# vlc-robot/robot-3dlotus

Hardware: AMD Instinct MI355X
Metric: keystep-samples/sec (train fwd+bwd) 3D-LOTUS GemBench (higher is better)
Workload: dtype f32; 1 GPU; 3D-LOTUS v1 (68.18M params), 16 key-step clouds x 4096 pts per GPU, fwd+loss+bwd, train mode (dropout on), fp32 exact (MFMA f32); global_batch=16, parallelism=dp1, rccl_ranks=0

## Files before the change

### robot-3dlotus_amd/csrc/conv.hip

```cpp
#include "mma.h"

namespace LOTUS_NS {

int lotus_reduce_parts(const float* part, float* out, long n, long stride, int nz, int accumulate, hipStream_t st);
int lotus_conv_pairs_try(int mode, const act_t* x, const float* w, const float* w_t, const float* bias, const act_t* add,
                         act_t* y, const int* nbr, const int* rowidx, int n, int T, int cin, int cout, void* workspace,
                         size_t workspace_bytes, int prec, hipStream_t st, int* rc);
size_t lotus_conv_pairs_workspace(int n, int ND);
int lotus_conv_weight_transpose_impl(const float* w, float* wt, int cout, int T, int cin, int prec, hipStream_t st);
int lotus_conv_tap_gemm(int mode, const act_t* x, const float* w, float* part, const int* tg_in, const int* tg_cnt, int n64,
                        int src_rows, int cin, int cout, hipStream_t st);

static int tap_min_width() {
  static int v = -1;
  if (v < 0) { const char* e = getenv("LOTUS_CONV_TAP_MINC"); v = e ? atoi(e) : 64; }
  return v;
}
static size_t tap_slab_max() {
  static long v = -1;
  if (v < 0) { const char* e = getenv("LOTUS_CONV_TAP_SLAB_MB"); v = e ? atol(e) : 2047; }
  return (size_t)v << 20;
}
static size_t tap_part_bytes(int n, int ND);
static bool tap_shape_ok(int n, int cin, int cout) {
// ... 386 lines not shown
      if (b_fast) rrb[e] = ldraw(p.x + (long)max(qq, 0) * p.cin + ci0 + iq * 4);
      else rrb[e] = toraw(load4_guard(p.x, p.cin, max(qq, 0), ci0 + iq * 4, p.n, p.cin, b_vec), p.x);
    }
  };
  auto stage = [&](unsigned* W, int plane, const float4& v0, const float4& v1, bool sum) __attribute__((always_inline)) {
    const float va[4] = {v0.x, v0.y, v0.z, v0.w}, vb[4] = {v1.x, v1.y, v1.z, v1.w};
    unsigned hw[4], lw[4];
#pragma unroll
    for (int e = 0; e < 4; ++e) split_bf16(va[e], vb[e], hw[e], lw[e]);
    if (sum) {
#pragma unroll
      for (int e = 0; e < 4; ++e) bsum[e] += va[e] + vb[e];
    }
    const int rot = (iq >> 2) & 3;
    rot4(hw, rot);
    if (PREC == 3) rot4(lw, rot);
#pragma unroll
    for (int e = 0; e < 4; ++e) {
      const int row = iq * 4 + ((e + rot) & 3);
      W[row * TA::kLdW + kr2] = hw[e];
      if (PREC == 3) W[plane + row * TA::kLdW + kr2] = lw[e];
    }
  };
  auto lstore = [&]() __attribute__((always_inline)) {
    stage(Aw, TA::kPlaneW, zsel4(oka[0], unraw(rra[0])), zsel4(oka[1], unraw(rra[1])), want_bias);
    stage(Bw, TB::kPlaneW, zsel4(okb[0], unraw(rrb[0])), zsel4(okb[1], unraw(rrb[1])), false);
  };
  if (total > 0) {
    gload(0);
    lstore();
    __syncthreads();
    for (int k0 = 0; k0 < total; k0 += BK) {
      const bool more = k0 + BK < total;
      if (more) gload(k0 + BK);
      gemm_slab_bf16<BM, BN, BK, PREC>(Aw, Bw, wr0, wc0, acc);
      __syncthreads();
      if (more) {
        lstore();
        __syncthreads();
      }
    }
  }
  float* part = p.part + (long)blockIdx.z * p.part_stride;
  const int col = ci0 + acc_col(wc0, 0);
  if (col < p.cin) {
#pragma unroll
    for (int r = 0; r < 16; ++r) {
      const int row = co0 + acc_row(wr0, 0, r);
      if (row < p.cout) part[((long)row * p.T + t) * p.cin + col] = acc[0][0][r];
    }
  }
  if (want_bias) {
    float4* red = reinterpret_cast<float4*>(Aw);
    red[tid] = make_float4(bsum[0], bsum[1], bsum[2], bsum[3]);
    __syncthreads();
    if (tid < BM) {
      float s = 0.f;
#pragma unroll
      for (int g = 0; g < 16; ++g) {
        const float4 v = red[g * 16 + (tid >> 2)];
        s += (tid & 3) == 0 ? v.x : (tid & 3) == 1 ? v.y : (tid & 3) == 2 ? v.z : v.w;
      }
      if (co0 + tid < p.cout) p.bias_part[(long)blockIdx.z * p.part_stride + co0 + tid] = s;
    }
  }
}

static size_t conv_dyn_lds(int T, int BM) { return (size_t)(T * BM + 2 * T) * sizeof(int); }

extern "C" {

size_t lotus_subm_conv_workspace(int n, int cin, int cout) {
  const size_t a = lotus_conv_pairs_workspace(n, cout), b = lotus_conv_pairs_workspace(n, cin);
  const size_t c = tap_shape_ok(n, cin, cout) ? tap_part_bytes(n, cin > cout ? cin : cout) : 0;
  const size_t ab = a > b ? a : b;
  return ab > c ? ab : c;
}
int lotus_conv_tap_eligible(int n, int cin, int cout) {
  static int on = -1;
  if (on < 0) { const char* e = getenv("LOTUS_CONV_TAP"); on = (e && e[0] == '0') ? 0 : 1; }
  return on && tap_shape_ok(n, cin, cout) ? 1 : 0;
}

#define STEM_ROWS 32
#define STEM_TP 128

}

__global__ void conv_stem_wt_kernel(const float* __restrict__ w, float* __restrict__ wt, int cout, int T, int cin) {
  const int i = blockIdx.x * blockDim.x + threadIdx.x;
  if (i >= cout * T * cin) return;
  const int c = i % cout, rem = i / cout;
  wt[i] = w[(long)c * T * cin + rem];
}

template <int CIN>
__global__ __launch_bounds__(256) void conv_smallcin_kernel(ConvP p) {
  __shared__ int list_nb[STEM_ROWS * STEM_TP];
  __shared__ unsigned char list_t[STEM_ROWS * STEM_TP];
  __shared__ int cnt_s[STEM_ROWS];
  const int tid = threadIdx.x, r = tid >> 3, j = tid & 7;
  const int m = blockIdx.y * STEM_ROWS + r, cb = blockIdx.x;
  const bool valid = m < p.n;
  {
    int nbv[16];
    unsigned flags = 0;
#pragma unroll
    for (int k = 0; k < 16; ++k) {
      const int t = 16 * j + k;
      nbv[k] = (valid && t < p.T) ? p.nbr[(long)t * p.n + m] : -1;
      flags |= (nbv[k] >= 0 ? 1u : 0u) << k;
    }
    const int mine = __popc(flags);
    int incl = mine;
#pragma unroll
    for (int o = 1; o < 8; o <<= 1) {
      const int v = __shfl_up(incl, o, 8);
      if (j >= o) incl += v;
    }
    int pos = incl - mine;
    if (j == 7) cnt_s[r] = incl;
#pragma unroll
    for (int k = 0; k < 16; ++k)
      if (flags & (1u << k)) {
        list_t[r * STEM_TP + pos] = (unsigned char)(16 * j + k);
        list_nb[r * STEM_TP + pos] = nbv[k];
        ++pos;
      }
  }
  float acc[8];
#pragma unroll
  for (int k = 0; k < 8; ++k) acc[k] = p.bias ? p.bias[cb * 64 + j * 8 + k] : 0.f;
  __syncthreads();
  const int len = cnt_s[r];
  const float* wbase = p.w + cb * 64 + j * 8;
  const int cin = CIN ? CIN : p.cin;
  int t = 0;
  float xl = 0.f;
  if (len > 0) {
    t = list_t[r * STEM_TP];
    xl = j < cin ? p.x[(long)list_nb[r * STEM_TP] * cin + j] : 0.f;
  }
  for (int cur = 0; cur < len; ++cur) {
    const float* wr = wbase + (long)t * cin * p.cout;
    const float xc = xl;
    if (cur + 1 < len) {
      t = list_t[r * STEM_TP + cur + 1];
      xl = j < cin ? p.x[(long)list_nb[r * STEM_TP + cur + 1] * cin + j] : 0.f;
    }
    if (CIN) {
      float4 w0[CIN ? CIN : 1], w1[CIN ? CIN : 1];
#pragma unroll
      for (int ci = 0; ci < CIN; ++ci) {
        w0[ci] = ld4(wr + ci * p.cout);
        w1[ci] = ld4(wr + ci * p.cout + 4);
      }
#pragma unroll
      for (int ci = 0; ci < CIN; ++ci) {
        const float xv = __shfl(xc, ci, 8);
        acc[0] = fmaf(xv, w0[ci].x, acc[0]); acc[1] = fmaf(xv, w0[ci].y, acc[1]); acc[2] = fmaf(xv, w0[ci].z, acc[2]); acc[3] = fmaf(xv, w0[ci].w, acc[3]);
        acc[4] = fmaf(xv, w1[ci].x, acc[4]); acc[5] = fmaf(xv, w1[ci].y, acc[5]); acc[6] = fmaf(xv, w1[ci].z, acc[6]); acc[7] = fmaf(xv, w1[ci].w, acc[7]);
      }
    } else {
      for (int ci = 0; ci < cin; ++ci) {
        const float4 w0 = ld4(wr + ci * p.cout);
        const float4 w1 = ld4(wr + ci * p.cout + 4);
        const float xv = __shfl(xc, ci, 8);
        acc[0] = fmaf(xv, w0.x, acc[0]); acc[1] = fmaf(xv, w0.y, acc[1]); acc[2] = fmaf(xv, w0.z, acc[2]); acc[3] = fmaf(xv, w0.w, acc[3]);
        acc[4] = fmaf(xv, w1.x, acc[4]); acc[5] = fmaf(xv, w1.y, acc[5]); acc[6] = fmaf(xv, w1.z, acc[6]); acc[7] = fmaf(xv, w1.w, acc[7]);
      }
    }
  }
  if (valid) {
    act_t* yo = p.y + (long)m * p.ND + cb * 64 + j * 8;
    if (p.add) {
      const act_t* ao = p.add + (long)m * p.ND + cb * 64 + j * 8;
#pragma unroll
      for (int k = 0; k < 8; ++k) acc[k] += ao[k];
    }
    st4(yo, make_float4(acc[0], acc[1], acc[2], acc[3]));
    st4(yo + 4, make_float4(acc[4], acc[5], acc[6], acc[7]));
  }
}

extern "C" {

int lotus_conv_weight_transpose(const float* w, float* w_t, int cout, int T, int cin, int precision, void* stream) {
  LOTUS_CHECK_ARG(w && w_t && cout > 0 && T > 0 && cin > 0, "lotus_conv_weight_transpose: bad arguments");
  LOTUS_CHECK_ARG(precision == 0 || precision == 1 || precision == 3, "lotus_conv_weight_transpose: precision must be 0, 1 or 3");
  return lotus_conv_weight_transpose_impl(w, w_t, cout, T, cin, precision, (hipStream_t)stream);
}

int lotus_subm_conv(int mode, const act_t* x, const float* w, const float* w_t, const float* bias, const act_t* add,
                    act_t* y, const int* nbr, const int* rowidx, int n, int T, int cin, int cout, int precision,
                    const int* tap_plan, void* workspace, size_t workspace_bytes, void* stream) {
  LOTUS_CHECK_ARG(x && w && y && nbr && n >= 0 && T > 0 && cin > 0 && cout > 0, "lotus_subm_conv: bad arguments");
  LOTUS_CHECK_ARG(precision == 0 || precision == 1 || precision == 3, "lotus_subm_conv: precision must be 0, 1 or 3");
  if (n == 0) return LOTUS_OK;
  if (tap_plan && T == 27 && precision == 0 && lotus_conv_tap_eligible(n, cin, cout)) {
    LOTUS_CHECK_ARG(workspace && ((uintptr_t)workspace) % 16 == 0 && workspace_bytes >= tap_part_bytes(n, mode == 0 ? cout : cin),
                    "lotus_subm_conv: the tap-grouped path needs a 16-byte aligned workspace of lotus_subm_conv_workspace(n, cin, cout) bytes");
    LOTUS_CHECK_ARG((((uintptr_t)x) | ((uintptr_t)w) | ((uintptr_t)y) | ((uintptr_t)bias) | ((uintptr_t)add)) % 16 == 0,
                    "lotus_subm_conv: the tap-grouped path needs 16-byte aligned operands");
    const int n64 = (n + 63) / 64 * 64, ND = mode == 0 ? cout : cin;
    const int rc = lotus_conv_tap_gemm(mode, x, w, (float*)workspace, tap_plan + 32, tap_plan, n64, n, cin, cout, (hipStream_t)stream);
    if (rc != LOTUS_OK) return rc;
    const long total4 = (long)n * ND / 4;
    const int g = (int)cdiv(total4, 256);
    LOTUS_LAUNCH(conv_tap_reduce_kernel, dim3(g > 4096 ? 4096 : g), dim3(256), 0, (hipStream_t)stream, (const float*)workspace,
                 tap_plan + 32 + 27L * n64, n, ND, bias, add, y);
    LOTUS_LAUNCH_CHECK("lotus_subm_conv(tap-grouped)");
    return LOTUS_OK;
  }
  {
    int rc = 0;
    if (lotus_conv_pairs_try(mode, x, w, w_t, bias, add, y, nbr, rowidx, n, T, cin, cout, workspace, workspace_bytes,
                             precision, (hipStream_t)stream, &rc))
      return rc;
  }
  ConvP p;
  memset(&p, 0, sizeof(p));
  p.x = x; p.w = w; p.y = y; p.bias = bias; p.add = add; p.nbr = nbr; p.rowidx = rowidx;
  p.n = n; p.T = T; p.cin = cin; p.cout = cout;
  p.KD = mode == 0 ? cin : cout;
  p.ND = mode == 0 ? cout : cin;
  p.mirror = mode == 1;
  hipStream_t st = (hipStream_t)stream;
  if (mode == 0 && cin <= 8 && cout % 64 == 0 && T <= STEM_TP && ((uintptr_t)y) % 16 == 0 && workspace &&
      ((uintptr_t)workspace) % 16 == 0 && workspace_bytes >= (size_t)T * cin * cout * sizeof(float)) {
    LOTUS_LAUNCH(conv_stem_wt_kernel, dim3(cdiv((long)cout * T * cin, 256)), dim3(256), 0, st, w, (float*)workspace, cout, T,
                       cin);
    p.w = (const float*)workspace;
    const dim3 sg(cout / 64, cdiv(n, STEM_ROWS));
    if (cin == 7) LOTUS_LAUNCH((conv_smallcin_kernel<7>), sg, dim3(256), 0, st, p);
    else if (cin == 8) LOTUS_LAUNCH((conv_smallcin_kernel<8>), sg, dim3(256), 0, st, p);
    else if (cin == 6) LOTUS_LAUNCH((conv_smallcin_kernel<6>), sg, dim3(256), 0, st, p);
    else if (cin == 4) LOTUS_LAUNCH((conv_smallcin_kernel<4>), sg, dim3(256), 0, st, p);
    else LOTUS_LAUNCH((conv_smallcin_kernel<0>), sg, dim3(256), 0, st, p);
    LOTUS_LAUNCH_CHECK("lotus_subm_conv(stem)");
    return LOTUS_OK;
  }
  dim3 block(256);
  const size_t dyn = conv_dyn_lds(T, 128);
  LOTUS_CHECK_ARG(dyn + 20000 <= 160 * 1024, "lotus_subm_conv: %d taps do not fit LDS", T);
  if (p.ND <= 64) {
    dim3 grid(cdiv(p.ND, 64), cdiv(n, 128));
    if (mode == 0) {
      { static bool a1 = false; if (!a1) { (void)hipFuncSetAttribute((const void*)conv_kernel<128, 64, true>, hipFuncAttributeMaxDynamicSharedMemorySize, (int)dyn); a1 = true; } }
      LOTUS_LAUNCH((conv_kernel<128, 64, true>), grid, block, dyn, st, p);
    } else {
      { static bool a2 = false; if (!a2) { (void)hipFuncSetAttribute((const void*)conv_kernel<128, 64, false>, hipFuncAttributeMaxDynamicSharedMemorySize, (int)dyn); a2 = true; } }
      LOTUS_LAUNCH((conv_kernel<128, 64, false>), grid, block, dyn, st, p);
    }
  } else {
    dim3 grid(cdiv(p.ND, 128), cdiv(n, 128));
    if (mode == 0) {
      { static bool a3 = false; if (!a3) { (void)hipFuncSetAttribute((const void*)conv_kernel<128, 128, true>, hipFuncAttributeMaxDynamicSharedMemorySize, (int)dyn); a3 = true; } }
      LOTUS_LAUNCH((conv_kernel<128, 128, true>), grid, block, dyn, st, p);
    } else {
      { static bool a4 = false; if (!a4) { (void)hipFuncSetAttribute((const void*)conv_kernel<128, 128, false>, hipFuncAttributeMaxDynamicSharedMemorySize, (int)dyn); a4 = true; } }
      LOTUS_LAUNCH((conv_kernel<128, 128, false>), grid, block, dyn, st, p);
    }
  }
  LOTUS_LAUNCH_CHECK("lotus_subm_conv");
  return LOTUS_OK;
}

static __global__ __launch_bounds__(256) void conv_smallcin_wgrad_kernel(ConvWgP p) {
  constexpr int NW = WG_MAX_PAIRS / 256, SB = 512;
  __shared__ int prow_s[WG_MAX_PAIRS];
  __shared__ int pnb_s[WG_MAX_PAIRS];
  __shared__ __attribute__((aligned(16))) float xs[SB][8];
  __shared__ float red[4][64][8];
  __shared__ int wcnt[NW][4];
  const int tid = threadIdx.x, c = tid & 63, g = tid >> 6, lane = tid & 63;
  const int cb = blockIdx.x, t = blockIdx.y, z = blockIdx.z;
  const int rbeg = z * p.chunk, rend = min(p.n, rbeg + p.chunk);
  int total = 0;
  {
    int nbv[NW];
    unsigned long long mv[NW];
#pragma unroll
    for (int w = 0; w < NW; ++w) {
      const int row = rbeg + w * 256 + tid;
      nbv[w] = row < rend ? p.nbr[(long)t * p.n + row] : -1;
    }
#pragma unroll
    for (int w = 0; w < NW; ++w) {
      mv[w] = __ballot(nbv[w] >= 0);
      if (lane == 0) wcnt[w][g] = __popcll(mv[w]);
    }
    __syncthreads();
#pragma unroll
    for (int w = 0; w < NW; ++w) {
      int base = total;
#pragma unroll
      for (int q = 0; q < 4; ++q) {
        if (q < g) base += wcnt[w][q];
        total += wcnt[w][q];
      }
      if (nbv[w] >= 0) {
        const int pos = base + __popcll(mv[w] & ((1ull << lane) - 1ull));
        prow_s[pos] = rbeg + w * 256 + tid;
        pnb_s[pos] = nbv[w];
      }
    }
  }
  __syncthreads();
  float acc[8];
#pragma unroll
  for (int k = 0; k < 8; ++k) acc[k] = 0.f;
  const act_t* dyc = p.dy + cb * 64 + c;
  for (int b0 = 0; b0 < total; b0 += SB) {
    const int nb = min(SB, total - b0);
#pragma unroll 4
    for (int i = tid; i < nb * 8; i += 256) {
      const int pi = i >> 3, ci = i & 7;
      xs[pi][ci] = ci < p.cin ? p.x[(long)pnb_s[b0 + pi] * p.cin + ci] : 0.f;
    }
    __syncthreads();
    int pi = g;
// ... 128 lines not shown
```

### robot-3dlotus_amd/csrc/pool_head.hip

```cpp
#include "common.h"

namespace LOTUS_NS {

int lotus_reduce_parts(const float* part, float* out, long n, long stride, int nz, int accumulate, hipStream_t st);

__global__ void pool_max_fwd_kernel(const act_t* __restrict__ x, const int* __restrict__ members,
                                    const int* __restrict__ seg, int nc, int C, act_t* __restrict__ y,
                                    int* __restrict__ arg) {
  LOTUS_T_PRIO();
  const int c4 = C / 4;
  const long gid = (long)blockIdx.x * blockDim.x + threadIdx.x;
  if (gid >= (long)nc * c4) return;
  const int c = (int)(gid / c4), q = (int)(gid % c4);
  const int a = seg[c], b = seg[c + 1];
  float best[4] = {-INFINITY, -INFINITY, -INFINITY, -INFINITY};
  int bi[4] = {-1, -1, -1, -1};
  for (int i = a; i < b; ++i) {
    const int p = members[i];
    const float4 v = ld4q(x + (long)p * C, q);
    const float vs[4] = {v.x, v.y, v.z, v.w};
#pragma unroll
    for (int e = 0; e < 4; ++e)
      if (vs[e] > best[e]) {
        best[e] = vs[e];
// ... 119 lines not shown
  const int4 a = reinterpret_cast<const int4*>(arg + (long)b * C)[q];
  float4 o = make_float4(a.x == p ? g.x : 0.f, a.y == p ? g.y : 0.f, a.z == p ? g.z : 0.f, a.w == p ? g.w : 0.f);
  if (add) {
    const float4 v = ld4q(add + (long)p * C, q);
    o.x += v.x; o.y += v.y; o.z += v.z; o.w += v.w;
  }
  st4q(dx + (long)p * C, q, o);
}

#define POS_CE_SPLITS 32
#define POS_CE_PART 8
__device__ __forceinline__ double wave_sum_d(double v) {
#pragma unroll
  for (int o = 32; o > 0; o >>= 1) v += __shfl_xor(v, o, 64);
  return v;
}
__global__ __launch_bounds__(256) void pos_ce_part_kernel(const act_t* __restrict__ xt, const float* __restrict__ tgt,
                                                          const int* __restrict__ off, int nb,
                                                          float* __restrict__ part ) {
  __shared__ float red[4];
  __shared__ double redd[4];
  const int s = blockIdx.x, bc = blockIdx.y, b = bc / 3, c = bc % 3;
  const int n0 = off[b], nn = off[b + 1] - n0;
  const int p0 = (int)((long)nn * s / POS_CE_SPLITS), p1 = (int)((long)nn * (s + 1) / POS_CE_SPLITS);
  const float* tb = tgt + (long)3 * nb * n0 + (long)c * nn * nb;
  const act_t* xb = xt + (long)n0 * (3 * nb) + c * nb;
  const int j0 = threadIdx.x & 31, g = threadIdx.x >> 5;
  float m = -INFINITY;
  for (int p = p0 + g; p < p1; p += 8)
    for (int j = j0; j < nb; j += 32) m = fmaxf(m, xb[(long)p * (3 * nb) + j]);
  m = wave_max(m);
  if ((threadIdx.x & 63) == 0) red[threadIdx.x >> 6] = m;
  __syncthreads();
  m = fmaxf(fmaxf(red[0], red[1]), fmaxf(red[2], red[3]));
  __syncthreads();
  double v[3] = {0.0, 0.0, 0.0};
  for (int p = p0 + g; p < p1; p += 8)
    for (int j = j0; j < nb; j += 32) {
      const float x = xb[(long)p * (3 * nb) + j], t = tb[(long)p * nb + j];
      v[0] += exp((double)x - (double)m);
      v[1] += (double)t * x;
      v[2] += t;
    }
  double tot[3];
#pragma unroll
  for (int k = 0; k < 3; ++k) {
    const double w = wave_sum_d(v[k]);
    if ((threadIdx.x & 63) == 0) redd[threadIdx.x >> 6] = w;
    __syncthreads();
    tot[k] = ((redd[0] + redd[1]) + redd[2]) + redd[3];
    __syncthreads();
  }
  if (threadIdx.x == 0) {
    float* o = part + ((long)bc * POS_CE_SPLITS + s) * POS_CE_PART;
    o[0] = m; o[1] = 0.f;
    double* od = reinterpret_cast<double*>(o + 2);
    od[0] = tot[0]; od[1] = tot[1]; od[2] = tot[2];
  }
}

__global__ __launch_bounds__(64) void pos_ce_merge_kernel(const float* __restrict__ part, float* __restrict__ stats) {
  const int bc = blockIdx.x, s = threadIdx.x;
  float m = -INFINITY;
  double se = 0.0, stx = 0.0, st = 0.0;
  if (s < POS_CE_SPLITS) {
    const float* o = part + ((long)bc * POS_CE_SPLITS + s) * POS_CE_PART;
    const double* od = reinterpret_cast<const double*>(o + 2);
    m = o[0]; se = od[0]; stx = od[1]; st = od[2];
  }
  const float M = wave_max(m);
  se = wave_sum_d(m > -INFINITY ? se * exp((double)m - (double)M) : 0.0);
  stx = wave_sum_d(stx);
  st = wave_sum_d(st);
  if (s == 0) {
    const double lse = (double)M + log(se);
    float* o = stats + (long)bc * 4;
    o[0] = (float)(lse * st - stx);
    o[1] = (float)lse;
    o[2] = (float)st;
    o[3] = (float)(lse - (double)o[1]);
  }
}

__global__ __launch_bounds__(256) void small_loss_kernel(const act_t* __restrict__ ae, const float* __restrict__ gt,
                                                         const float* __restrict__ pos_stats, int B, int nrot, int ga,
                                                         float pos_w, float rot_w, float* __restrict__ losses,
                                                         float* __restrict__ dae) {
  __shared__ float acc[3];
  const int W = nrot * 3 + 1;
  if (threadIdx.x < 3) acc[threadIdx.x] = 0.f;
  __syncthreads();
  float rot = 0.f, opn = 0.f, pos = 0.f;
  for (int i = threadIdx.x; i < B * 3; i += 256) {
    const int b = i / 3, a = i % 3;
    const act_t* row = ae + (long)b * W;
    float m = -INFINITY;
    for (int k = 0; k < nrot; ++k) m = fmaxf(m, row[k * 3 + a]);
    float se = 0.f;
    for (int k = 0; k < nrot; ++k) se += expf(row[k * 3 + a] - m);
    const float lse = m + logf(se);
    const int tk = (int)gt[(long)b * ga + 3 + a];
    rot += lse - row[tk * 3 + a];
    if (dae)
      for (int k = 0; k < nrot; ++k)
        dae[(long)b * W + k * 3 + a] = (expf(row[k * 3 + a] - lse) - (k == tk ? 1.f : 0.f)) / (B * 3);
    pos += pos_stats[(long)i * 4];
  }
  for (int b = threadIdx.x; b < B; b += 256) {
    const float x = ae[(long)b * W + W - 1], t = gt[(long)b * ga + ga - 1];
    opn += fmaxf(x, 0.f) - x * t + log1pf(expf(-fabsf(x)));
    if (dae) dae[(long)b * W + W - 1] = (1.f / (1.f + expf(-x)) - t) / B;
  }
  __shared__ float red[3][4];
  float v3[3] = {pos, rot, opn};
#pragma unroll
  for (int k = 0; k < 3; ++k) {
    const float w = wave_sum(v3[k]);
    if ((threadIdx.x & 63) == 0) red[k][threadIdx.x >> 6] = w;
  }
  __syncthreads();
  if (threadIdx.x == 0) {
    for (int k = 0; k < 3; ++k) acc[k] = ((red[k][0] + red[k][1]) + red[k][2]) + red[k][3];
    const float lp = acc[0] / (3.f * B), lr = acc[1] / (3.f * B), lo = acc[2] / B;
    losses[0] = lp; losses[1] = lr; losses[2] = lo; losses[3] = pos_w * lp + rot_w * lr + lo;
  }
}

__global__ void pos_ce_bwd_kernel(const act_t* __restrict__ xt, const float* __restrict__ tgt,
                                  const int* __restrict__ off, const int* __restrict__ batch,
                                  const float* __restrict__ stats, const float* __restrict__ gl, float pos_w, int B,
                                  int n, int nb, act_t* __restrict__ dxt) {
  const long gid = (long)blockIdx.x * blockDim.x + threadIdx.x;
  const long total = (long)n * 3 * nb;
  if (gid >= total) return;
  const int p = (int)(gid / (3 * nb)), rem = (int)(gid % (3 * nb)), c = rem / nb, bin = rem % nb;
  const int b = batch[p];
  const int n0 = off[b], nn = off[b + 1] - n0;
  const float t = tgt[(long)3 * nb * n0 + (long)c * nn * nb + (long)(p - n0) * nb + bin];
  const float* s = stats + (long)(b * 3 + c) * 4;
  const float coef = (gl[0] + pos_w * gl[3]) / (3.f * B);
  dxt[gid] = (float)((double)coef * (exp((double)xt[gid] - ((double)s[1] + (double)s[3])) * (double)s[2] - (double)t));
}

__global__ void pos_ce_bwd_w_kernel(const act_t* __restrict__ xt, const float* __restrict__ tgt,
                                    const int* __restrict__ off, const int* __restrict__ batch,
                                    const float* __restrict__ stats, const float* __restrict__ g, int n, int nb,
                                    act_t* __restrict__ dxt) {
  const long gid = (long)blockIdx.x * blockDim.x + threadIdx.x;
  const long total = (long)n * 3 * nb;
  if (gid >= total) return;
  const int p = (int)(gid / (3 * nb)), rem = (int)(gid % (3 * nb)), c = rem / nb, bin = rem % nb;
  const int b = batch[p];
  const int n0 = off[b], nn = off[b + 1] - n0;
  const float t = tgt[(long)3 * nb * n0 + (long)c * nn * nb + (long)(p - n0) * nb + bin];
  const float* s = stats + (long)(b * 3 + c) * 4;
  dxt[gid] = (float)((double)g[b * 3 + c] * (exp((double)xt[gid] - ((double)s[1] + (double)s[3])) * (double)s[2] - (double)t));
}

__global__ void ae_grad_kernel(const float* __restrict__ x, const float* __restrict__ gl, float rot_w, int W, long n,
                               act_t* __restrict__ y) {
  const long i = (long)blockIdx.x * blockDim.x + threadIdx.x;
  if (i >= n) return;
  const bool open_col = (i % W) == W - 1;
  y[i] = x[i] * (open_col ? gl[2] + gl[3] : gl[1] + rot_w * gl[3]);
}

__global__ __launch_bounds__(256) void mp_loss_kernel(const act_t* __restrict__ ae, const float* __restrict__ gt,
                                                      const float* __restrict__ stop, const float* __restrict__ mask,
                                                      const float* __restrict__ ce, int B, int T, int nrot, int ga, float pos_w,
                                                      float rot_w, float* __restrict__ losses, float* __restrict__ dae,
                                                      float* __restrict__ dce) {
  extern __shared__ float msum_b[];
  __shared__ float red[4][4];
  __shared__ float msum_s;
  const int W = nrot * 3 + 2, R = B * T, tid = threadIdx.x;
  for (int b = tid; b < B; b += 256) {
    float s = 0.f;
    for (int t = 0; t < T; ++t) s += mask[b * T + t];
    msum_b[b] = s;
  }
  __syncthreads();
  if (tid == 0) {
    float s = 0.f;
    for (int b = 0; b < B; ++b) s += msum_b[b];
    msum_s = s;
  }
  __syncthreads();
  const float msum = msum_s;
  float pos = 0.f, rot = 0.f, opn = 0.f, stp = 0.f;
  for (int i = tid; i < R * 3; i += 256) {
    const int r = i / 3, a = i % 3, b = r / T;
    const float m = mask[r];
    const act_t* row = ae + (long)r * W;
    float mx = -INFINITY;
    for (int k = 0; k < nrot; ++k) mx = fmaxf(mx, row[k * 3 + a]);
    float se = 0.f;
    for (int k = 0; k < nrot; ++k) se += expf(row[k * 3 + a] - mx);
    const float lse = mx + logf(se);
    const int tk = (int)gt[(long)r * ga + 3 + a];
    rot += (lse - row[tk * 3 + a]) * m;
    const float sc = m / msum / 3.f;
// ... 239 lines not shown
  if (threadIdx.x) return;
  float best = -INFINITY;
  long bi = 0x7fffffffffffffffL;
  for (int s = 0; s < PT_SPLITS; ++s) {
    const double* o = part + ((long)bc * PT_SPLITS + s) * 3;
    pick_max(best, bi, (float)o[0], (long)o[1]);
  }
  if (off[b + 1] == off[b]) { best_pos[bc] = 0.0; return; }
  const long p = bi / nb;
  const int j = (int)(bi % nb);
  best_pos[bc] = cand_coord(j - nb / 2, bin, (double)pc[(long)(off[b] + p) * ld + c]);
}

extern "C" {

int lotus_pool_max_fwd(const act_t* x, const int* members, const int* seg, int nc, int C, act_t* y, int* arg,
                       void* stream) {
  LOTUS_CHECK_ARG(x && members && seg && y && arg && C % 4 == 0, "lotus_pool_max_fwd: bad arguments");
  if (nc == 0) return LOTUS_OK;
  LOTUS_LAUNCH(pool_max_fwd_kernel, dim3(cdiv((long)nc * C / 4, 256)), dim3(256), 0, (hipStream_t)stream, x,
                     members, seg, nc, C, y, arg);
  LOTUS_LAUNCH_CHECK("lotus_pool_max_fwd");
  return LOTUS_OK;
}
int lotus_pool_max_bwd(const act_t* dy, const int* arg, const int* cluster, int n, int C, act_t* dx, void* stream) {
  LOTUS_CHECK_ARG(dy && arg && cluster && dx && C % 4 == 0, "lotus_pool_max_bwd: bad arguments");
  if (n == 0) return LOTUS_OK;
  LOTUS_LAUNCH(pool_max_bwd_kernel, dim3(cdiv((long)n * C / 4, 256)), dim3(256), 0, (hipStream_t)stream, dy, arg,
                     cluster, n, C, dx);
  LOTUS_LAUNCH_CHECK("lotus_pool_max_bwd");
  return LOTUS_OK;
}
int lotus_unpool_fwd(const act_t* skip, const act_t* up, const int* cluster, int n, int C, act_t* x, void* stream) {
  LOTUS_CHECK_ARG(skip && up && cluster && x && C % 4 == 0, "lotus_unpool_fwd: bad arguments");
  if (n == 0) return LOTUS_OK;
  LOTUS_LAUNCH(unpool_fwd_kernel, dim3(cdiv((long)n * C / 4, 256)), dim3(256), 0, (hipStream_t)stream, skip, up,
                     cluster, n, C, x);
  LOTUS_LAUNCH_CHECK("lotus_unpool_fwd");
  return LOTUS_OK;
}
int lotus_unpool_bwd(const act_t* dx, const int* members, const int* seg, int nc, int C, act_t* dup, void* stream) {
  LOTUS_CHECK_ARG(dx && members && seg && dup && C % 4 == 0, "lotus_unpool_bwd: bad arguments");
  if (nc == 0) return LOTUS_OK;
  LOTUS_LAUNCH(unpool_bwd_kernel, dim3(cdiv((long)nc * C / 4, 256)), dim3(256), 0, (hipStream_t)stream, dx,
                     members, seg, nc, C, dup);
  LOTUS_LAUNCH_CHECK("lotus_unpool_bwd");
  return LOTUS_OK;
}
size_t lotus_cloud_max_workspace(int B, int C) { return (size_t)B * CM_SPLITS * C * (sizeof(float) + sizeof(int)); }
int lotus_cloud_max_fwd(const act_t* x, const int* off, int B, int C, act_t* y, int* arg, void* workspace, size_t workspace_bytes,
                        void* stream) {
  LOTUS_CHECK_ARG(x && off && y && arg && B > 0 && C > 0 && C % 4 == 0 && ((uintptr_t)x) % 16 == 0,
                  "lotus_cloud_max_fwd: bad arguments (C must be a multiple of 4, x 16-byte aligned)");
  LOTUS_CHECK_ARG(workspace && ((uintptr_t)workspace) % 16 == 0 && workspace_bytes >= lotus_cloud_max_workspace(B, C),
                  "lotus_cloud_max_fwd: workspace too small");
  float* pv = (float*)workspace;
  int* pi = (int*)(pv + (size_t)B * CM_SPLITS * C);
  hipStream_t st = (hipStream_t)stream;
  LOTUS_LAUNCH(cloud_max_part_kernel, dim3(B, cdiv(C, 128), CM_SPLITS), dim3(1024), 0, st, x, off, C, pv, pi);
  LOTUS_LAUNCH(cloud_max_merge_kernel, dim3(cdiv(B * C, 256)), dim3(256), 0, st, (const float*)pv, (const int*)pi, B, C, y, arg);
  LOTUS_LAUNCH_CHECK("lotus_cloud_max_fwd");
  return LOTUS_OK;
}
int lotus_cloud_max_bwd(const act_t* dy, const int* arg, const int* batch, int n, int C, const act_t* add, act_t* dx,
                        void* stream) {
  LOTUS_CHECK_ARG(dy && arg && batch && dx && C % 4 == 0, "lotus_cloud_max_bwd: bad arguments");
  if (n == 0) return LOTUS_OK;
  LOTUS_LAUNCH(cloud_max_bwd_kernel, dim3(cdiv((long)n * C / 4, 256)), dim3(256), 0, (hipStream_t)stream, dy, arg,
                     batch, n, C, add, dx);
  LOTUS_LAUNCH_CHECK("lotus_cloud_max_bwd");
  return LOTUS_OK;
}

size_t lotus_loss_stats_floats(int B) { return (size_t)B * 3 * (4 + POS_CE_PART * POS_CE_SPLITS); }

int lotus_loss_fwd(const act_t* xt, const act_t* ae, const float* tgt, const float* gt, const int* off, int B, int nb,
                   int nrot, int ga, float pos_w, float rot_w, float* losses, float* pos_stats, float* dae,
                   void* stream) {
  LOTUS_CHECK_ARG(xt && ae && tgt && gt && off && losses && pos_stats && B > 0, "lotus_loss_fwd: bad arguments");
  hipStream_t st = (hipStream_t)stream;
  float* part = pos_stats + (size_t)B * 3 * 4;
  LOTUS_LAUNCH(pos_ce_part_kernel, dim3(POS_CE_SPLITS, B * 3), dim3(256), 0, st, xt, tgt, off, nb, part);
  LOTUS_LAUNCH(pos_ce_merge_kernel, dim3(B * 3), dim3(64), 0, st, (const float*)part, pos_stats);
  LOTUS_LAUNCH(small_loss_kernel, dim3(1), dim3(256), 0, st, ae, gt, pos_stats, B, nrot, ga, pos_w, rot_w, losses, dae);
  LOTUS_LAUNCH_CHECK("lotus_loss_fwd");
  return LOTUS_OK;
}
int lotus_loss_bwd(const act_t* xt, const float* tgt, const int* off, const int* batch, const float* pos_stats,
                   const float* dae_saved, const float* gl, float pos_w, float rot_w, int B, int n, int nb, int nrot,
                   act_t* dxt, act_t* dae_out, void* stream) {
  LOTUS_CHECK_ARG(xt && tgt && off && batch && pos_stats && dae_saved && gl && dxt && dae_out, "lotus_loss_bwd: bad arguments");
  hipStream_t st = (hipStream_t)stream;
  const long total = (long)n * 3 * nb;
  LOTUS_LAUNCH(pos_ce_bwd_kernel, dim3(cdiv(total, 256)), dim3(256), 0, st, xt, tgt, off, batch, pos_stats, gl,
                     pos_w, B, n, nb, dxt);
  const int W = nrot * 3 + 1;
  LOTUS_LAUNCH(ae_grad_kernel, dim3(cdiv((long)B * W, 256)), dim3(256), 0, st, dae_saved, gl, rot_w, W,
                     (long)B * W, dae_out);
  LOTUS_LAUNCH_CHECK("lotus_loss_bwd");
  return LOTUS_OK;
}

int lotus_pos_ce_fwd(const act_t* xt, const float* tgt, const int* off, int B, int nb, float* pos_stats, void* stream) {
  LOTUS_CHECK_ARG(xt && tgt && off && pos_stats && B > 0 && nb > 0, "lotus_pos_ce_fwd: bad arguments");
  hipStream_t st = (hipStream_t)stream;
  float* part = pos_stats + (size_t)B * 3 * 4;
  LOTUS_LAUNCH(pos_ce_part_kernel, dim3(POS_CE_SPLITS, B * 3), dim3(256), 0, st, xt, tgt, off, nb, part);
  LOTUS_LAUNCH(pos_ce_merge_kernel, dim3(B * 3), dim3(64), 0, st, (const float*)part, pos_stats);
  LOTUS_LAUNCH_CHECK("lotus_pos_ce_fwd");
  return LOTUS_OK;
}
int lotus_pos_ce_bwd(const act_t* xt, const float* tgt, const int* off, const int* batch, const float* pos_stats,
                     const float* g, int B, int n, int nb, act_t* dxt, void* stream) {
  LOTUS_CHECK_ARG(xt && tgt && off && batch && pos_stats && g && dxt && B > 0, "lotus_pos_ce_bwd: bad arguments");
  if (n == 0) return LOTUS_OK;
  const long total = (long)n * 3 * nb;
  LOTUS_LAUNCH(pos_ce_bwd_w_kernel, dim3(cdiv(total, 256)), dim3(256), 0, (hipStream_t)stream, xt, tgt, off, batch,
                     pos_stats, g, n, nb, dxt);
  LOTUS_LAUNCH_CHECK("lotus_pos_ce_bwd");
  return LOTUS_OK;
}

int lotus_mp_loss_fwd(const act_t* ae, const float* gt, const float* stop, const float* mask, const float* ce, int B, int T,
                      int nrot, int ga, float pos_w, float rot_w, float* losses, float* dae, float* dce, void* stream) {
  LOTUS_CHECK_ARG(ae && gt && stop && mask && ce && losses && dae && dce && B > 0 && T > 0 && nrot > 0 && ga >= 7 && B <= 8192,
                  "lotus_mp_loss_fwd: bad arguments");
  LOTUS_LAUNCH(mp_loss_kernel, dim3(1), dim3(256), (size_t)B * sizeof(float), (hipStream_t)stream, ae, gt, stop, mask, ce, B, T,
               nrot, ga, pos_w, rot_w, losses, dae, dce);
  LOTUS_LAUNCH_CHECK("lotus_mp_loss_fwd");
  return LOTUS_OK;
}
int lotus_mp_loss_bwd(const float* dae, const float* dce, const float* g, float pos_w, float rot_w, int B, int T, int nrot,
                      act_t* dae_out, float* dce_out, void* stream) {
  LOTUS_CHECK_ARG(dae && dce && g && dae_out && dce_out && B > 0 && T > 0 && nrot > 0, "lotus_mp_loss_bwd: bad arguments");
  const int W = nrot * 3 + 2;
  const long nae = (long)B * T * W, nce = (long)B * T * 3;
  LOTUS_LAUNCH(mp_loss_bwd_kernel, dim3(cdiv(nae, 256)), dim3(256), 0, (hipStream_t)stream, dae, dce, g, pos_w, rot_w, W, nae, nce,
               dae_out, dce_out);
  LOTUS_LAUNCH_CHECK("lotus_mp_loss_bwd");
  return LOTUS_OK;
}

int lotus_add(const act_t* a, const act_t* b, act_t* y, long n, void* stream) {
  LOTUS_CHECK_ARG(a && b && y && n % 4 == 0, "lotus_add: bad arguments");
  if (n == 0) return LOTUS_OK;
  int g = cdiv(n / 4, 256);
  LOTUS_LAUNCH(add_kernel, dim3(g > 4096 ? 4096 : g), dim3(256), 0, (hipStream_t)stream, a, b, y, n / 4);
  LOTUS_LAUNCH_CHECK("lotus_add");
  return LOTUS_OK;
}
int lotus_dropout(const act_t* x, act_t* y, long n, float p, unsigned long long seed, void* stream) {
  LOTUS_CHECK_ARG(x && y && p >= 0.f && p < 1.f, "lotus_dropout: bad arguments");
  if (n == 0) return LOTUS_OK;
  unsigned th; float inv;
  lotus_drop_setup(p, &th, &inv);
  int g = cdiv(n, 256);
  LOTUS_LAUNCH(dropout_mask_kernel, dim3(g > 4096 ? 4096 : g), dim3(256), 0, (hipStream_t)stream, x, y, n, seed, th, inv);
  LOTUS_LAUNCH_CHECK("lotus_dropout");
  return LOTUS_OK;
}

int lotus_drop_path(const act_t* branch, const act_t* x, act_t* y, int M, int C, float p, unsigned long long seed, void* stream) {
  LOTUS_CHECK_ARG(branch && y && M >= 0 && C > 0 && C % 4 == 0 && p >= 0.f && p < 1.f, "lotus_drop_path: bad arguments");
  if (M == 0) return LOTUS_OK;
  unsigned th; float inv;
  lotus_drop_setup(p, &th, &inv);
  const long total4 = (long)M * (C / 4);
// ... 77 lines not shown
```

Before: 1082 keystep-samples/s.

## Restructure stem conv to stage weights in LDS and parallelize rotation loss per wave

The small-cin stem convolution is rewritten so each block of 8 waves covers 128 rows. Weight tiles for 16 taps are staged in shared memory with a register prefetch of the next tile. Each lane owns one output channel, and neighbor features are broadcast with readlane, replacing per-row compaction and repeated global weight loads. Separately, the single-block rotation cross-entropy loss kernel now runs with 1024 threads and assigns one wave per item with wave-level max and sum reductions. This trades serial per-thread loops for more sync and readlane overhead.

New measurement: 1090 keystep-samples/s (median of 6 runs). Within noise of the previous version (+0.7%).

```diff
diff --git a/robot-3dlotus_amd/csrc/conv.hip b/robot-3dlotus_amd/csrc/conv.hip
--- a/robot-3dlotus_amd/csrc/conv.hip
+++ b/robot-3dlotus_amd/csrc/conv.hip
@@ -492,7 +492,11 @@
   return on && tap_shape_ok(n, cin, cout) ? 1 : 0;
 }
 
-#define STEM_ROWS 32
+#define STEM_WAVES 8
+#define STEM_R 16
+#define STEM_ROWS (STEM_WAVES * STEM_R)
+#define STEM_XT 8
+#define STEM_WT 16
 #define STEM_TP 128
 
 }
@@ -505,91 +509,107 @@
 }
 
 template <int CIN>
-__global__ __launch_bounds__(256) void conv_smallcin_kernel(ConvP p) {
-  __shared__ int list_nb[STEM_ROWS * STEM_TP];
-  __shared__ unsigned char list_t[STEM_ROWS * STEM_TP];
-  __shared__ int cnt_s[STEM_ROWS];
-  const int tid = threadIdx.x, r = tid >> 3, j = tid & 7;
-  const int m = blockIdx.y * STEM_ROWS + r, cb = blockIdx.x;
-  const bool valid = m < p.n;
+__global__ __launch_bounds__(STEM_WAVES * 64) void conv_smallcin_kernel(ConvP p) {
+  __shared__ __attribute__((aligned(16))) float w_s[STEM_WT * 8 * 64];
+  const int tid = threadIdx.x, lane = tid & 63, wv = tid >> 6;
+  const int cin = CIN ? CIN : p.cin;
+  const int cb = blockIdx.x;
+  const int row0 = blockIdx.y * STEM_ROWS + wv * STEM_R;
+  const int er = lane & (STEM_R - 1), eq = lane >> 4;
+  const int m_e = row0 + er;
+  const int NX = (p.T + STEM_XT - 1) / STEM_XT;
+  const int wrows_all = p.T * cin;
+
+  auto load_nb = [&](int i, int (&nb)[2]) {
+#pragma unroll
+    for (int k = 0; k < 2; ++k) {
+      const int t = i * STEM_XT + 4 * k + eq;
+      nb[k] = (i < NX && t < p.T && m_e < p.n) ? p.nbr[(long)t * p.n + m_e] : -1;
+    }
+  };
+  auto load_x = [&](const int (&nb)[2], float (&xr)[2][8]) {
+#pragma unroll
+    for (int k = 0; k < 2; ++k)
+#pragma unroll
+      for (int ci = 0; ci < 8; ++ci) xr[k][ci] = (ci < cin && nb[k] >= 0) ? ld1(p.x + (long)nb[k] * cin + ci) : 0.f;
+  };
+  auto load_w = [&](int s, float4 (&wr)[4]) {
+    const int r0 = s * STEM_WT * cin, nr = min(STEM_WT * cin, wrows_all - r0);
+#pragma unroll
+    for (int k = 0; k < 4; ++k) {
+      const int idx = k * (STEM_WAVES * 64) + tid, rw = idx >> 4, c4 = idx & 15;
+      wr[k] = rw < nr ? ld4(p.w + (long)(r0 + rw) * p.cout + cb * 64 + c4 * 4) : make_float4(0.f, 0.f, 0.f, 0.f);
+    }
+  };
+
+  float acc[STEM_R];
   {
-    int nbv[16];
-    unsigned flags = 0;
-#pragma unroll
-    for (int k = 0; k < 16; ++k) {
-      const int t = 16 * j + k;
-      nbv[k] = (valid && t < p.T) ? p.nbr[(long)t * p.n + m] : -1;
-      flags |= (nbv[k] >= 0 ? 1u : 0u) << k;
-    }
-    const int mine = __popc(flags);
-    int incl = mine;
-#pragma unroll
-    for (int o = 1; o < 8; o <<= 1) {
-      const int v = __shfl_up(incl, o, 8);
-      if (j >= o) incl += v;
-    }
-    int pos = incl - mine;
-    if (j == 7) cnt_s[r] = incl;
-#pragma unroll
-    for (int k = 0; k < 16; ++k)
-      if (flags & (1u << k)) {
-        list_t[r * STEM_TP + pos] = (unsigned char)(16 * j + k);
-        list_nb[r * STEM_TP + pos] = nbv[k];
-        ++pos;
-      }
-  }
-  float acc[8];
-#pragma unroll
-  for (int k = 0; k < 8; ++k) acc[k] = p.bias ? p.bias[cb * 64 + j * 8 + k] : 0.f;
-  __syncthreads();
-  const int len = cnt_s[r];
-  const float* wbase = p.w + cb * 64 + j * 8;
-  const int cin = CIN ? CIN : p.cin;
-  int t = 0;
-  float xl = 0.f;
-  if (len > 0) {
-    t = list_t[r * STEM_TP];
-    xl = j < cin ? p.x[(long)list_nb[r * STEM_TP] * cin + j] : 0.f;
-  }
-  for (int cur = 0; cur < len; ++cur) {
-    const float* wr = wbase + (long)t * cin * p.cout;
-    const float xc = xl;
-    if (cur + 1 < len) {
-      t = list_t[r * STEM_TP + cur + 1];
-      xl = j < cin ? p.x[(long)list_nb[r * STEM_TP + cur + 1] * cin + j] : 0.f;
-    }
-    if (CIN) {
-      float4 w0[CIN ? CIN : 1], w1[CIN ? CIN : 1];
-#pragma unroll
-      for (int ci = 0; ci < CIN; ++ci) {
-        w0[ci] = ld4(wr + ci * p.cout);
-        w1[ci] = ld4(wr + ci * p.cout + 4);
-      }
-#pragma unroll
-      for (int ci = 0; ci < CIN; ++ci) {
-        const float xv = __shfl(xc, ci, 8);
-        acc[0] = fmaf(xv, w0[ci].x, acc[0]); acc[1] = fmaf(xv, w0[ci].y, acc[1]); acc[2] = fmaf(xv, w0[ci].z, acc[2]); acc[3] = fmaf(xv, w0[ci].w, acc[3]);
-        acc[4] = fmaf(xv, w1[ci].x, acc[4]); acc[5] = fmaf(xv, w1[ci].y, acc[5]); acc[6] = fmaf(xv, w1[ci].z, acc[6]); acc[7] = fmaf(xv, w1[ci].w, acc[7]);
-      }
-    } else {
-      for (int ci = 0; ci < cin; ++ci) {
-        const float4 w0 = ld4(wr + ci * p.cout);
-        const float4 w1 = ld4(wr + ci * p.cout + 4);
-        const float xv = __shfl(xc, ci, 8);
-        acc[0] = fmaf(xv, w0.x, acc[0]); acc[1] = fmaf(xv, w0.y, acc[1]); acc[2] = fmaf(xv, w0.z, acc[2]); acc[3] = fmaf(xv, w0.w, acc[3]);
-        acc[4] = fmaf(xv, w1.x, acc[4]); acc[5] = fmaf(xv, w1.y, acc[5]); acc[6] = fmaf(xv, w1.z, acc[6]); acc[7] = fmaf(xv, w1.w, acc[7]);
-      }
-    }
-  }
-  if (valid) {
-    act_t* yo = p.y + (long)m * p.ND + cb * 64 + j * 8;
-    if (p.add) {
-      const act_t* ao = p.add + (long)m * p.ND + cb * 64 + j * 8;
-#pragma unroll
-      for (int k = 0; k < 8; ++k) acc[k] += ao[k];
-    }
-    st4(yo, make_float4(acc[0], acc[1], acc[2], acc[3]));
-    st4(yo + 4, make_float4(acc[4], acc[5], acc[6], acc[7]));
+    const float b0 = p.bias ? p.bias[cb * 64 + lane] : 0.f;
+#pragma unroll
+    for (int r = 0; r < STEM_R; ++r) acc[r] = b0;
+  }
+  int nb_cur[2], nb_nxt[2];
+  float xr[2][8];
+  float4 wr[4];
+  load_w(0, wr);
+  load_nb(0, nb_cur);
+  load_nb(1, nb_nxt);
+  load_x(nb_cur, xr);
+
+#pragma unroll 1
+  for (int i = 0; i < NX; ++i) {
+    if ((i & 1) == 0) {
+      __syncthreads();
+#pragma unroll
+      for (int k = 0; k < 4; ++k) {
+        const int idx = k * (STEM_WAVES * 64) + tid;
+        st4(w_s + (idx >> 4) * 64 + (idx & 15) * 4, wr[k]);
+      }
+      __syncthreads();
+      load_w((i >> 1) + 1, wr);
+    }
+    const unsigned long long bal0 = __ballot(nb_cur[0] >= 0), bal1 = __ballot(nb_cur[1] >= 0);
+    float xc[2][8];
+#pragma unroll
+    for (int k = 0; k < 2; ++k)
+#pragma unroll
+      for (int ci = 0; ci < 8; ++ci) {
+        xc[k][ci] = xr[k][ci];
+        if (ci < cin) asm volatile("" : "+v"(xc[k][ci]));
+      }
+    nb_cur[0] = nb_nxt[0]; nb_cur[1] = nb_nxt[1];
+    load_x(nb_cur, xr);
+    load_nb(i + 2, nb_nxt);
+
+    const float* wst = w_s + (i & 1) * STEM_XT * cin * 64 + lane;
+#pragma unroll
+    for (int q = 0; q < STEM_XT; ++q) {
+      const unsigned mk = (unsigned)((q < 4 ? bal0 : bal1) >> (16 * (q & 3))) & 0xffffu;
+      if (mk == 0) continue;
+      float wq[8];
+#pragma unroll
+      for (int ci = 0; ci < 8; ++ci) wq[ci] = ci < cin ? wst[(q * cin + ci) * 64] : 0.f;
+#pragma unroll
+      for (int r = 0; r < STEM_R; ++r) {
+        if (!((mk >> r) & 1u)) continue;
+        const int src = (q & 3) * STEM_R + r;
+        float a = acc[r];
+#pragma unroll
+        for (int ci = 0; ci < 8; ++ci)
+          if (ci < cin) a = fmaf(__int_as_float(__builtin_amdgcn_readlane(__float_as_int(xc[q >> 2][ci]), src)), wq[ci], a);
+        acc[r] = a;
+      }
+    }
+  }
+#pragma unroll
+  for (int r = 0; r < STEM_R; ++r) {
+    const int m = row0 + r;
+    if (m < p.n) {
+      const long o = (long)m * p.ND + cb * 64 + lane;
+      float a = acc[r];
+      if (p.add) a += ld1(p.add + o);
+      st1(p.y + o, a);
+    }
   }
 }
 
@@ -642,11 +662,12 @@
                        cin);
     p.w = (const float*)workspace;
     const dim3 sg(cout / 64, cdiv(n, STEM_ROWS));
-    if (cin == 7) LOTUS_LAUNCH((conv_smallcin_kernel<7>), sg, dim3(256), 0, st, p);
-    else if (cin == 8) LOTUS_LAUNCH((conv_smallcin_kernel<8>), sg, dim3(256), 0, st, p);
-    else if (cin == 6) LOTUS_LAUNCH((conv_smallcin_kernel<6>), sg, dim3(256), 0, st, p);
-    else if (cin == 4) LOTUS_LAUNCH((conv_smallcin_kernel<4>), sg, dim3(256), 0, st, p);
-    else LOTUS_LAUNCH((conv_smallcin_kernel<0>), sg, dim3(256), 0, st, p);
+    const dim3 sb(STEM_WAVES * 64);
+    if (cin == 7) LOTUS_LAUNCH((conv_smallcin_kernel<7>), sg, sb, 0, st, p);
+    else if (cin == 8) LOTUS_LAUNCH((conv_smallcin_kernel<8>), sg, sb, 0, st, p);
+    else if (cin == 6) LOTUS_LAUNCH((conv_smallcin_kernel<6>), sg, sb, 0, st, p);
+    else if (cin == 4) LOTUS_LAUNCH((conv_smallcin_kernel<4>), sg, sb, 0, st, p);
+    else LOTUS_LAUNCH((conv_smallcin_kernel<0>), sg, sb, 0, st, p);
     LOTUS_LAUNCH_CHECK("lotus_subm_conv(stem)");
     return LOTUS_OK;
   }
diff --git a/robot-3dlotus_amd/csrc/pool_head.hip b/robot-3dlotus_amd/csrc/pool_head.hip
--- a/robot-3dlotus_amd/csrc/pool_head.hip
+++ b/robot-3dlotus_amd/csrc/pool_head.hip
@@ -225,41 +225,91 @@
   }
 }
 
-__global__ __launch_bounds__(256) void small_loss_kernel(const act_t* __restrict__ ae, const float* __restrict__ gt,
-                                                         const float* __restrict__ pos_stats, int B, int nrot, int ga,
-                                                         float pos_w, float rot_w, float* __restrict__ losses,
-                                                         float* __restrict__ dae) {
+__global__ __launch_bounds__(1024) void small_loss_kernel(const act_t* __restrict__ ae, const float* __restrict__ gt,
+                                                          const float* __restrict__ pos_stats, int B, int nrot, int ga,
+                                                          float pos_w, float rot_w, float* __restrict__ losses,
+                                                          float* __restrict__ dae) {
   __shared__ float acc[3];
+  __shared__ float item_s[256];
   const int W = nrot * 3 + 1;
+  const int lane = threadIdx.x & 63, wv = threadIdx.x >> 6, nwv = blockDim.x >> 6;
   if (threadIdx.x < 3) acc[threadIdx.x] = 0.f;
   __syncthreads();
   float rot = 0.f, opn = 0.f, pos = 0.f;
-  for (int i = threadIdx.x; i < B * 3; i += 256) {
-    const int b = i / 3, a = i % 3;
-    const act_t* row = ae + (long)b * W;
-    float m = -INFINITY;
-    for (int k = 0; k < nrot; ++k) m = fmaxf(m, row[k * 3 + a]);
-    float se = 0.f;
-    for (int k = 0; k < nrot; ++k) se += expf(row[k * 3 + a] - m);
-    const float lse = m + logf(se);
-    const int tk = (int)gt[(long)b * ga + 3 + a];
-    rot += lse - row[tk * 3 + a];
-    if (dae)
-      for (int k = 0; k < nrot; ++k)
-        dae[(long)b * W + k * 3 + a] = (expf(row[k * 3 + a] - lse) - (k == tk ? 1.f : 0.f)) / (B * 3);
-    pos += pos_stats[(long)i * 4];
-  }
-  for (int b = threadIdx.x; b < B; b += 256) {
-    const float x = ae[(long)b * W + W - 1], t = gt[(long)b * ga + ga - 1];
-    opn += fmaxf(x, 0.f) - x * t + log1pf(expf(-fabsf(x)));
-    if (dae) dae[(long)b * W + W - 1] = (1.f / (1.f + expf(-x)) - t) / B;
-  }
+  const bool own = threadIdx.x < 256;
+  const float ps0 = own && threadIdx.x < B * 3 ? pos_stats[(long)threadIdx.x * 4] : 0.f;
+  float ox0 = 0.f, ot0 = 0.f;
+  if (own && threadIdx.x < B) { ox0 = ae[(long)threadIdx.x * W + W - 1]; ot0 = gt[(long)threadIdx.x * ga + ga - 1]; }
+  const bool inreg = nrot <= 128;
+  auto fetch = [&](int i, float& v0, float& v1, float& g) {
+    v0 = v1 = -INFINITY; g = 0.f;
+    if (i < B * 3) {
+      const act_t* row = ae + (long)(i / 3) * W + i % 3;
+      if (lane < nrot) v0 = row[lane * 3];
+      if (lane + 64 < nrot) v1 = row[(lane + 64) * 3];
+      g = gt[(long)(i / 3) * ga + 3 + i % 3];
+    }
+  };
+  for (int base = 0; base < B * 3; base += 256) {
+    const int iend = min(B * 3, base + 256);
+    float n0, n1, ng;
+    if (inreg) fetch(base + wv < iend ? base + wv : B * 3, n0, n1, ng);
+    for (int i = base + wv; i < iend; i += nwv) {
+      const int b = i / 3, a = i % 3;
+      const act_t* row = ae + (long)b * W;
+      if (inreg) {
+        const float v0 = n0, v1 = n1;
+        const int tk = __builtin_amdgcn_readfirstlane((int)ng);
+        fetch(i + nwv < iend ? i + nwv : B * 3, n0, n1, ng);
+        const float m = wave_max(fmaxf(v0, v1));
+        const float e0 = lane < nrot ? expf(v0 - m) : 0.f, e1 = lane + 64 < nrot ? expf(v1 - m) : 0.f;
+        float se = 0.f;
+        for (int l = 0; l < min(64, nrot); ++l) se += __int_as_float(__builtin_amdgcn_readlane(__float_as_int(e0), l));
+        for (int l = 0; l < nrot - 64; ++l) se += __int_as_float(__builtin_amdgcn_readlane(__float_as_int(e1), l));
+        const float lse = m + logf(se);
+        const float vt = __int_as_float(__builtin_amdgcn_readlane(__float_as_int(tk < 64 ? v0 : v1), tk & 63));
+        if (lane == 0) item_s[i - base] = lse - vt;
+        if (dae) {
+          if (lane < nrot) dae[(long)b * W + lane * 3 + a] = (expf(v0 - lse) - (lane == tk ? 1.f : 0.f)) / (B * 3);
+          if (lane + 64 < nrot) dae[(long)b * W + (lane + 64) * 3 + a] = (expf(v1 - lse) - (lane + 64 == tk ? 1.f : 0.f)) / (B * 3);
+        }
+        continue;
+      }
+      float m = -INFINITY;
+      for (int k = lane; k < nrot; k += 64) m = fmaxf(m, row[k * 3 + a]);
+      m = wave_max(m);
+      float se = 0.f;
+      for (int k0 = 0; k0 < nrot; k0 += 64) {
+        const float e = k0 + lane < nrot ? expf(row[(k0 + lane) * 3 + a] - m) : 0.f;
+        const int cnt = min(64, nrot - k0);
+        for (int l = 0; l < cnt; ++l) se += __int_as_float(__builtin_amdgcn_readlane(__float_as_int(e), l));
+      }
+      const float lse = m + logf(se);
+      const int tk = (int)gt[(long)b * ga + 3 + a];
+      if (lane == 0) item_s[i - base] = lse - row[tk * 3 + a];
+      if (dae)
+        for (int k = lane; k < nrot; k += 64)
+          dae[(long)b * W + k * 3 + a] = (expf(row[k * 3 + a] - lse) - (k == tk ? 1.f : 0.f)) / (B * 3);
+    }
+    __syncthreads();
+    if (own && base + threadIdx.x < B * 3) {
+      rot += item_s[threadIdx.x];
+      pos += base ? pos_stats[(long)(base + threadIdx.x) * 4] : ps0;
+    }
+    __syncthreads();
+  }
+  if (own)
+    for (int b = threadIdx.x; b < B; b += 256) {
+      const float x = b < 256 ? ox0 : (float)ae[(long)b * W + W - 1], t = b < 256 ? ot0 : gt[(long)b * ga + ga - 1];
+      opn += fmaxf(x, 0.f) - x * t + log1pf(expf(-fabsf(x)));
+      if (dae) dae[(long)b * W + W - 1] = (1.f / (1.f + expf(-x)) - t) / B;
+    }
   __shared__ float red[3][4];
   float v3[3] = {pos, rot, opn};
 #pragma unroll
   for (int k = 0; k < 3; ++k) {
     const float w = wave_sum(v3[k]);
-    if ((threadIdx.x & 63) == 0) red[k][threadIdx.x >> 6] = w;
+    if ((threadIdx.x & 63) == 0 && threadIdx.x < 256) red[k][threadIdx.x >> 6] = w;
   }
   __syncthreads();
   if (threadIdx.x == 0) {
@@ -665,7 +715,7 @@
   float* part = pos_stats + (size_t)B * 3 * 4;
   LOTUS_LAUNCH(pos_ce_part_kernel, dim3(POS_CE_SPLITS, B * 3), dim3(256), 0, st, xt, tgt, off, nb, part);
   LOTUS_LAUNCH(pos_ce_merge_kernel, dim3(B * 3), dim3(64), 0, st, (const float*)part, pos_stats);
-  LOTUS_LAUNCH(small_loss_kernel, dim3(1), dim3(256), 0, st, ae, gt, pos_stats, B, nrot, ga, pos_w, rot_w, losses, dae);
+  LOTUS_LAUNCH(small_loss_kernel, dim3(1), dim3(1024), 0, st, ae, gt, pos_stats, B, nrot, ga, pos_w, rot_w, losses, dae);
   LOTUS_LAUNCH_CHECK("lotus_loss_fwd");
   return LOTUS_OK;
 }
```
